# jturner65/distRayTracer_old

Measured on AMD Instinct MI355X. Metric: Mray/s + achieved HBM GB/s, bun69k.cli 1024² 16spp, 1/2/4/8 GPU, higher is better.
Workload: dtype f64

## Files before the change

distraytracer_old_amd/csrc/scene_build.cpp:

```cpp
#include <algorithm>
#include <cmath>
#include <map>
#include <string>

#include "host_math.h"
#include "rt_internal.h"

namespace rt {
using namespace hm;

namespace {

struct Box {
  double mn[3] = {100000, 100000, 100000};
  double mx[3] = {-100000, -100000, -100000};
};
static void calc_min_max(Box& b, const double* mn, const double* mx) {
  for (int i = 0; i < 3; ++i) { b.mn[i] = jmin(mn[i], b.mn[i]); b.mx[i] = jmax(mx[i], b.mx[i]); }
}
static void expand_pt(Box& b, D3 p) {
  double v[3] = {p.x, p.y, p.z};
  for (int i = 0; i < 3; ++i) {
    b.mn[i] = (b.mn[i] < v[i]) ? b.mn[i] : v[i];
    b.mx[i] = (b.mx[i] > v[i]) ? b.mx[i] : v[i];
// ... 451 lines not shown
        if (s.num_colors < 4) { err = "stone: needs at least 4 noise colours (mortar pair + a brick pair)"; return false; }
        md.distFunc = s.dist_func; md.roiFunc = s.roi_func; md.numPtsDist = s.num_pts_dist; md.mortar = s.mortar_thresh;
        std::map<double, int> pdfs;
        double lastDist = 1.0 / std::pow(M_E, s.avg_per_cell), cumProb = lastDist;
        for (int i = 1; i < 15; ++i) {
          lastDist *= (s.avg_per_cell / (1.0 * i));
          cumProb += lastDist;
          pdfs[cumProb] = i;
        }
        md.npdf = 0;
        for (auto& e : pdfs) { md.pdfKey[md.npdf] = e.first; md.pdfVal[md.npdf] = e.second; md.npdf++; }
      }
      hs.mat.push_back(md);
    }
    for (int l = 0; l < d->num_lights; ++l) {
      const rt_light_desc& s = d->lights[l];
      LightD ld;
      std::memset(&ld, 0, sizeof(ld));
      ld.type = s.type;
      ld.index = l;
      for (int c = 0; c < 3; ++c) { ld.origin[c] = s.pos[c]; ld.color[c] = s.color[c]; }
      D3 o = normalized(d3(s.dir[0], s.dir[1], s.dir[2]));
      ld.orient[0] = o.x; ld.orient[1] = o.y; ld.orient[2] = o.z;
      if (s.type != RT_LIGHT_POINT) {
        D3 t = ortho(o);
        ld.tangent[0] = t.x; ld.tangent[1] = t.y; ld.tangent[2] = t.z;
      }
      ld.innerRad = s.inner_deg * DEG_TO_RAD_F;
      ld.outerRad = s.outer_deg * DEG_TO_RAD_F;
      ld.radDiff = ld.outerRad - ld.innerRad;
      ld.radius = s.radius;
      std::memcpy(ld.g, s.ctm, sizeof(ld.g));
      {
        bool ident = true;
        for (int q = 0; q < 16; ++q) ident = ident && ld.g[q] == ((q % 5 == 0) ? 1.0 : 0.0);
        ld.pad[0] = (ident && (s.type == RT_LIGHT_POINT || s.type == RT_LIGHT_SPOT)) ? 1 : 0;
      }
      hs.light.push_back(ld);
    }
    int64_t off = 0;
    for (int t = 0; t < d->num_textures; ++t) {
      const rt_texture_desc& s = d->textures[t];
      if (s.w <= 0 || s.h <= 0 || !s.rgb) { err = "bad texture"; return false; }
      TexD td;
      td.w = s.w; td.h = s.h; td.off = off;
      hs.tex.push_back(td);
      for (int64_t k = 0; k < (int64_t)s.w * s.h; ++k)
        hs.texel.push_back(0xFF000000u | ((uint32_t)s.rgb[3 * k] << 16) | ((uint32_t)s.rgb[3 * k + 1] << 8) | s.rgb[3 * k + 2]);
      off += (int64_t)s.w * s.h;
    }
    if (d->bkg_texture >= d->num_textures) { err = "bad background texture"; return false; }
    hs.fov = d->fov;
    for (int c = 0; c < 3; ++c) hs.bg[c] = d->background[c];
    hs.bkgTex = d->bkg_texture;
    for (int c = 0; c < 4; ++c) hs.sky[c] = d->skydome[c];
    hs.dof = d->dof; hs.lensRadius = d->lens_radius; hs.lensFocal = d->lens_focal;
    if (d->camera < RT_CAMERA_FOV || d->camera > RT_CAMERA_ORTHO) { err = "bad camera type"; return false; }
    hs.camera = d->camera;
    hs.cameraParam[0] = d->camera_param[0]; hs.cameraParam[1] = d->camera_param[1];
    if (hs.camera != RT_CAMERA_FOV) hs.dof = 0;
    hs.rpp = d->rays_per_pixel;
    hs.photonMode = d->photon_mode; hs.photonCount = d->photon_count; hs.photonK = d->photon_k;
    hs.photonMaxD2 = d->photon_max_dist * d->photon_max_dist;
    return true;
  }
};

// ... 119 lines not shown
```

distraytracer_old_amd/csrc/trace_device.h:

```cpp
#pragma once
#include <hip/hip_runtime.h>
#include <stdint.h>

#include "rt_types.h"
#define QD_FN __device__ __forceinline__
#include "qdiv.h"

namespace rt {
namespace dv {

#define DEVI __device__ __forceinline__

static constexpr double EPS = 0.0000001;
static constexpr double DMAX = 1.7976931348623157e308;
static constexpr double TWO_PI_F = 6.2831854820251465;
static constexpr double PI_F = 3.1415927410125732;
static constexpr double PI_D = 3.141592653589793;

enum : uint32_t {
  SITE_AA_Y = 1, SITE_AA_X = 2, SITE_DOF_ANG = 3, SITE_DOF_RAD = 4, SITE_TIME = 8,
  SITE_DISK = 0x100, SITE_SHADOW_TIME = 0x200, SITE_PH_DIR = 0x1000, SITE_PH_BOUNCE = 0x1100, SITE_PH_TIME = 0x1200
};
enum { C_CAMERA = 0, C_SHADOW, C_REFL, C_REFR, C_BOX, C_TRI, C_QUAD, C_IMPLICIT, C_LIGHT, C_PHOTON, C_TEXEL,
       C_NODE, C_LEAF, C_MEMBER, C_ROOT, C_TOP,
       C_WNODE, C_WTRI, C_WQUAD, C_WIMPLICIT, C_WLIGHT, C_WPHOTON, C_N = 24 };

struct V {
  double x, y, z;
};
DEVI V mk(double x, double y, double z) { V r; r.x = x; r.y = y; r.z = z; return r; }
DEVI V sub(V a, V b) { return mk(a.x - b.x, a.y - b.y, a.z - b.z); }
DEVI V add(V a, V b) { return mk(a.x + b.x, a.y + b.y, a.z + b.z); }
DEVI V scl(V a, double s) { return mk(a.x * s, a.y * s, a.z * s); }
DEVI double dot(V a, V b) { return ((a.x * b.x) + (a.y * b.y)) + (a.z * b.z); }
DEVI V cross(V a, V b) { return mk((a.y * b.z) - (a.z * b.y), (a.z * b.x) - (a.x * b.z), (a.x * b.y) - (a.y * b.x)); }
DEVI double mag(V a) { return sqrt(((a.x * a.x) + (a.y * a.y)) + (a.z * a.z)); }
DEVI V nrmz(V a) {
  double m = mag(a);
  if (m == 0) return a;
  return mk(a.x / m, a.y / m, a.z / m);
}
DEVI bool veq(V a, V b) { return a.x == b.x && a.y == b.y && a.z == b.z; }
DEVI V ld3(const double* p) { return mk(p[0], p[1], p[2]); }
DEVI double jmin(double a, double b) { return (a != a) ? a : ((a <= b) ? a : b); }
DEVI double jmax(double a, double b) { return (a != a) ? a : ((a >= b) ? a : b); }
DEVI int32_t jd2i(double v) {
  if (v != v) return 0;
  if (v >= 2147483647.0) return 2147483647;
  if (v <= -2147483648.0) return (int32_t)0x80000000;
  return (int32_t)v;
}
DEVI V xpt(const double* m, V p) {
  double r[3];
#pragma unroll
  for (int row = 0; row < 3; ++row) {
    double a = 0.0;
    a += m[row * 4 + 0] * p.x;
    a += m[row * 4 + 1] * p.y;
    a += m[row * 4 + 2] * p.z;
    a += m[row * 4 + 3] * 1.0;
    r[row] = a;
  }
  return mk(r[0], r[1], r[2]);
}
DEVI V xvec(const double* m, V p) {
  double r[3];
#pragma unroll
  for (int row = 0; row < 3; ++row) {
    double a = 0.0;
    a += m[row * 4 + 0] * p.x;
    a += m[row * 4 + 1] * p.y;
    a += m[row * 4 + 2] * p.z;
    a += m[row * 4 + 3] * 0.0;
    r[row] = a;
  }
  return mk(r[0], r[1], r[2]);
}

DEVI uint64_t mix64(uint64_t z) {
  z += 0x9E3779B97F4A7C15ULL;
  z = (z ^ (z >> 30)) * 0xBF58476D1CE4E5B9ULL;
  z = (z ^ (z >> 27)) * 0x94D049BB133111EBULL;
  return z ^ (z >> 31);
}
DEVI double rng(uint64_t seed, uint64_t a, uint32_t b, uint32_t c, uint32_t site, uint32_t k, double lo, double hi) {
  uint64_t h = mix64(seed ^ mix64(a));
  h = mix64(h ^ (((uint64_t)b << 32) | c));
  h = mix64(h ^ (((uint64_t)site << 32) | k));
  double r = (double)(h >> 11) * 0x1.0p-53;
  r = r * (hi - lo) + lo;
  if (r >= hi) r = __longlong_as_double(__double_as_longlong(hi) - 1);
  return r;
}

struct Key {
  uint64_t seed, pixel;
  uint32_t sample, node;
  uint32_t tsite;
};

struct WRay {
  V o, d, d0;
  uint32_t ver;
  bool stable;
  bool moved;
};
DEVI void renorm(WRay& r) {
  if (!r.stable) {
    V n = nrmz(r.d);
    r.stable = veq(n, r.d);
    if (!r.stable) { r.moved = true; r.ver++; }
    r.d = n;
  }
}

#ifdef RT_PROF_PKSTAT
enum { P_CB_STEP = C_N, P_CB_LANES, P_CT_STEP, P_CT_LANES, P_AB_STEP, P_AB_LANES, P_AT_STEP, P_AT_LANES,
       P_RAY_STEP, P_RAY_LANES, P_SH_STEP, P_SH_LANES,
       P_CTH_STEP, P_CTH_LANES, P_ATH_STEP, P_ATH_LANES,
       P_N };
#else
enum { P_N = C_N };
#endif
struct Counters {
  uint64_t c[P_N];
};

struct RayInv {
  double y[3];
  bool fast;
};
DEVI RayInv ray_inv(V o, V d, int sceneOk) {
  RayInv r;
  r.y[0] = 1.0 / d.x; r.y[1] = 1.0 / d.y; r.y[2] = 1.0 / d.z;
  r.fast = sceneOk && qd_range(d.x) && qd_range(d.y) && qd_range(d.z) && qc_range(o.x) && qc_range(o.y) && qc_range(o.z);
  return r;
}

template <bool FAST>
DEVI bool slab_t(const double* mn, const double* mx, V o, V d, const double* y, double& tEntry) {
  double ro[3] = {o.x, o.y, o.z}, rd[3] = {d.x, d.y, d.z};
// ... 137 lines not shown
    if (r == 1) {
      const double g = (dist - te) - EPS, tol = APX * (fabs(te) + fabs(dist));
      if (g > tol) return true;
      if (-g > tol) return false;
    }
  }
  return slab_exact(mn, mx, o, d, ri, te) && (dist - te) > EPS;
}

DEVI int slab_plane(const double* mn, const double* mx, V o, V d) {
  double ro[3] = {o.x, o.y, o.z}, rd[3] = {d.x, d.y, d.z};
  double biggestMin = -DMAX;
  int idx = -1;
  for (int i = 0; i < 3; ++i) {
    double t1 = (mn[i] - ro[i]) / rd[i], t2 = (mx[i] - ro[i]) / rd[i];
    if (t1 < t2) { if (biggestMin < t1) { idx = i; biggestMin = t1; } }
    else { if (biggestMin < t2) { idx = i + 3; biggestMin = t2; } }
  }
  return idx;
}

struct LimNone {
  DEVI bool ok(double) const { return true; }
};
struct LimClosest {
  double a, b;
  DEVI bool ok(double t) const { return t < a || t < b; }
};
struct LimShadow {
  double dist;
  DEVI bool ok(double t) const { return (dist - t) > EPS; }
};

template <int NV, bool PLANE, class LIM = LimNone>
DEVI bool planar_test(const double (*v)[3], V nA, V nB, double dA, double dB, V o, V d, double& t, int& st,
                      const LIM& lim = LIM()) {
  double pr = dot(nA, d);
  if (!(fabs(pr) > 0)) return false;
  V N;
  double D;
  if (pr > 0) {
    pr = dot(nB, d);
    if (!(fabs(pr) > 0) || pr > 0) return false;
    N = nB; D = dB; st = 1;
  } else {
    N = nA; D = dA; st = 0;
  }
  t = -(dot(N, o) + D) / pr;
  if (!(t > EPS)) return false;
  if (PLANE) return true;
  if (!lim.ok(t)) return false;
  V p = mk(d.x * t + o.x, d.y * t + o.y, d.z * t + o.z);
#pragma unroll
  for (int i = 0; i < NV; ++i) {
    int vi = st ? (NV - 1 - i) : i;
    int pi = st ? (NV - 1 - (i == 0 ? NV - 1 : i - 1)) : (i == 0 ? NV - 1 : i - 1);
    V w = ld3(v[vi]), wp = ld3(v[pi]);
    V e = sub(w, wp);
    V ir = mk(p.x - w.x, p.y - w.y, p.z - w.z);
    if (dot(cross(ir, e), N) < -EPS) return false;
  }
  return true;
}

template <class LIM = LimNone, class TR = TriD>
DEVI bool tri_test(const TR& T, V o, V d, double& t, int& st, const LIM& lim = LIM()) {
  V nA = ld3(T.n);
  V nB = mk(-nA.x, -nA.y, -nA.z);
  return planar_test<3, false>(T.v, nA, nB, T.dA, T.dB, o, d, t, st, lim);
}

template <bool SL, class T>
DEVI T pld(const T* p) {
  if constexpr (SL) return *(const __attribute__((address_space(4))) T*)p;
  else return *p;
}
template <bool SL>
DEVI V pld3(const double* p) { return mk(pld<SL>(p), pld<SL>(p + 1), pld<SL>(p + 2)); }

template <bool SL = false>
DEVI V sphere_center(const PrimD& P, const Key& k) {
  if (pld<SL>(&P.type) != PT_MSPHERE) return pld3<SL>(P.a);
  double tm = rng(k.seed, k.pixel, k.sample, k.node, k.tsite, pld<SL>(&P.key), 0, 1.0);
  V o0 = pld3<SL>(P.a), o1 = pld3<SL>(P.a + 6);
  V bMa = sub(o1, o0);
  return mk(o0.x + tm * bMa.x, o0.y + tm * bMa.y, o0.z + tm * bMa.z);
}

template <bool SL = false>
DEVI bool prim_test(const PrimD& P, V o, V d, const Key& k, double& t, int& args) {
  const int32_t type = pld<SL>(&P.type);
  auto A = [&](int i) { return pld<SL>(P.a + i); };
  switch (type) {
    case PT_QUAD:
    case PT_PLANE: {
      if constexpr (SL) {
        double q[4][3];
#pragma unroll
        for (int i = 0; i < 12; ++i) q[i / 3][i % 3] = A(i);
        if (type == PT_PLANE)
          return planar_test<4, true>(q, pld3<SL>(P.a + 12), pld3<SL>(P.a + 15), A(18), A(19), o, d, t, args);
        return planar_test<4, false>(q, pld3<SL>(P.a + 12), pld3<SL>(P.a + 15), A(18), A(19), o, d, t, args);
// ... 110 lines not shown
```

distraytracer_old_amd/csrc/trace_kernels.h:

```cpp
#pragma once
#include "trace_device.h"
#include "jfdlibm.h"

namespace rt {
namespace dv {

enum : uint32_t {
  FT_PRIM = 1,
  FT_TEX = 2,
  FT_PHOTON = 4,
  FT_TRANS = 8,
  FT_DOF = 16,
  FT_LIGHTX = 32,
  FT_CAMX = 64,
  FT_INST = 128,
  FT_PASS = 256,
  FT_CELL = 512,
  FT_ALL = 1023
};

static __constant__ int c_perm[256];
static __constant__ int c_grad3[12][3];

struct Best {
  double t;
  int32_t ref;
  uint32_t ver;
  int16_t top;
  int16_t inAcc;
  int32_t inst;
  uint32_t iver;
};
DEVI Best miss() { Best b; b.t = DMAX; b.ref = 0; b.top = -1; b.ver = 0; b.inAcc = 0; b.inst = -1; b.iver = 0; return b; }
struct HitCtx {
  int32_t top, inst;
  uint32_t wver;
};

#define WCNT(idx, n)                                                                      \
  do {                                                                                    \
    if (CNT && __lane_id() == (int)__builtin_ctzll(__ballot(1))) ct.c[idx] += (n);        \
  } while (0)
#ifndef RT_ULOAD
#define RT_ULOAD 1
#endif
#ifndef RT_SPRIM
#define RT_SPRIM 2
#endif
template <uint32_t F>
static constexpr bool SPRIM = RT_SPRIM == 2 || (RT_SPRIM == 1 && (F & FT_PHOTON) == 0);
template <bool CNT, uint32_t F, class LIM = LimNone, bool WAVE = false>
DEVI bool test_ref(const SceneD& S, int32_t ref, V o, V d, const Key& k, double& t, int& args, Counters& ct,
                   const LIM& lim = LIM()) {
  if (!(F & FT_PRIM) || ref >= 0) {
    if (CNT) ct.c[C_TRI]++;
    if (WAVE) WCNT(C_WTRI, 1); else if (CNT) ct.c[C_WTRI]++;
    return tri_test(S.tri[ref], o, d, t, args, lim);
  }
  const PrimD& P = S.prim[~ref];
  if (CNT) {
    const int c = (P.type == PT_QUAD || P.type == PT_PLANE) ? C_QUAD : C_IMPLICIT;
    ct.c[c]++;
    if (WAVE) WCNT(c + (C_WQUAD - C_QUAD), 1); else ct.c[c + (C_WQUAD - C_QUAD)]++;
  }
  return prim_test<WAVE && SPRIM<F>>(P, o, d, k, t, args);
}
template <uint32_t F>
DEVI int32_t ref_xf(const SceneD& S, int32_t ref) { return (!(F & FT_PRIM) || ref >= 0) ? S.tri[ref].xf : S.prim[~ref].xf; }

template <class T>
DEVI T sload(const T* p) {
  static_assert(sizeof(T) == 4 || sizeof(T) == 8, "scalar field");
  return *(const __attribute__((address_space(4))) T*)p;
}
struct ChildBox {
  double mn[3], mx[3];
  int32_t ref;
};
DEVI ChildBox sload_child(const NodeD* nd, int side) {
  ChildBox c;
  const double* b = side ? nd->rmin : nd->lmin;
#pragma unroll
  for (int i = 0; i < 3; ++i) { c.mn[i] = sload(b + i); c.mx[i] = sload(b + 3 + i); }
  c.ref = sload(side ? &nd->right : &nd->left);
  return c;
}
struct TriG {
  double v[3][3];
  double n[3];
  double dA, dB;
// ... 120 lines not shown
#pragma unroll
  for (int i = 0; i < 9; ++i) t.m[i] = sload(&p->m[0][0] + i);
#pragma unroll
  for (int i = 0; i < 3; ++i) { t.c[i] = sload(p->c + i); t.n[i] = sload(p->n + i); }
  t.d = sload(&p->d); t.k = sload(&p->k); t.tm = sload(&p->tm);
  return t;
}
static constexpr float EPS_F32_UP = 1.00000001168609742e-07f;
DEVI bool tri_f32_out(const TriFR& T, const TriRayF& r) {
  const float s = __builtin_fmaf(T.n[2], r.d[2], __builtin_fmaf(T.n[1], r.d[1], T.n[0] * r.d[0]));
  const float P = __builtin_fmaf(T.n[2], r.o[2], __builtin_fmaf(T.n[1], r.o[1], __builtin_fmaf(T.n[0], r.o[0], T.d)));
  const float as = fabsf(s), sP = s < 0 ? -P : P;
  const float B = __builtin_fmaf(r.D, __builtin_fmaf(T.k, r.O + T.tm, 0x1p-40f), 0x1p-100f);
  const float thr = -__builtin_fmaf(EPS_F32_UP, as, B);
  bool out = false;
#pragma unroll
  for (int j = 0; j < 3; ++j) {
    const float* m = T.m + 3 * j;
    const float Q = __builtin_fmaf(m[2], r.o[2], __builtin_fmaf(m[1], r.o[1], __builtin_fmaf(m[0], r.o[0], -T.c[j])));
    const float R = __builtin_fmaf(m[2], r.d[2], __builtin_fmaf(m[1], r.d[1], m[0] * r.d[0]));
    out = out || (__builtin_fmaf(as, Q, -(sP * R)) < thr);
  }
  return out && as > 0x1p-20f * r.D && B < 0x1p100f;
}

template <bool CNT, uint32_t F, bool PK, class LIM = LimNone>
DEVI bool test_ref_u(const SceneD& S, int32_t ref, V o, V d, const Key& k, double& t, int& args, Counters& ct,
                     const LIM& lim = LIM()) {
  if constexpr (PK) {
    if (!(F & FT_PRIM) || ref >= 0) {
      if (CNT) ct.c[C_TRI]++;
      WCNT(C_WTRI, 1);
      const TriG T = sload_tri(S.tri + ref);
      return tri_test(T, o, d, t, args, lim);
    }
  }
  return test_ref<CNT, F, LIM, PK>(S, ref, o, d, k, t, args, ct, lim);
}
template <uint32_t F, bool PK>
DEVI int32_t ref_xf_u(const SceneD& S, int32_t ref) {
  if (PK && (!(F & FT_PRIM) || ref >= 0)) return sload(&S.tri[ref].xf);
  return ref_xf<F>(S, ref);
}
template <uint32_t F>
DEVI bool is_inst(const SceneD& S, int32_t ref) { return (F & FT_INST) && ref < 0 && S.prim[~ref].type == PT_INST; }


struct LeafR {
  int32_t start, count;
  bool run;
};
template <bool PK = false>
DEVI LeafR leaf_of(const SceneD& S, int32_t c) {
  LeafR r;
  r.run = (c & LEAF_RUN_FLAG) != 0;
  if (r.run) { r.start = (c >> 5) & LEAF_RUN_MAXSTART; r.count = c & 31; }
  else if (PK) { r.start = sload(&S.leaf[c].start); r.count = sload(&S.leaf[c].count); }
  else { LeafD lf = S.leaf[c]; r.start = lf.start; r.count = lf.count; }
  return r;
}
template <bool PK = false>
DEVI int32_t leaf_member(const SceneD& S, const LeafR& lf, int i) {
  return lf.run ? lf.start + i : (PK ? sload(S.member + lf.start + i) : S.member[lf.start + i]);
}

template <bool CNT, uint32_t F>
DEVI void inst_closest(const SceneD& S, int32_t ii, WRay& w, const Key& k, int top, Best& best, double& local, Counters& ct);

template <bool CNT, uint32_t F, bool INST, bool PK = false>
DEVI void leaf_closest(const SceneD& S, int32_t leaf, int accXf, V ao, V ad, WRay& w, const Key& k, const HitCtx& hc,
                       Best& best, double& local, Counters& ct) {
  const LeafR lf = leaf_of<PK>(S, leaf);
  if (CNT) { ct.c[C_LEAF]++; ct.c[C_MEMBER] += lf.count; }
  constexpr bool TF32 = PK && !INST && RT_F32_TRI != 0 && RT_F32_TRI_CPK != 0 &&
                        ((F & FT_PHOTON) == 0 || RT_F32_TRI_PH_CPK != 0);
  TriRayF trf;
  if constexpr (TF32) trf = tri_ray_f32(ao, ad);
  for (int i = 0; i < lf.count; ++i) {
    if (PK) PKSTAT(P_CT_STEP, __ballot(1));
    int32_t ref = leaf_member<PK>(S, lf, i);
    renorm(w);
    if constexpr (!INST && (F & FT_INST) != 0) {
      if (is_inst<F>(S, ref)) {
        inst_closest<CNT, F>(S, ~ref, w, k, hc.top, best, local, ct);
        continue;
      }
    }
    int xf = ref_xf_u<F, PK>(S, ref);
    V o, d;
    if (xf == accXf && !w.moved) { o = ao; d = ad; }
    else if (PK && (RT_ULOAD & 1)) {
      double inv[12];
      sload_inv(S.xf + xf, inv);
      o = xpt(inv, w.o); d = xvec(inv, w.d);
    } else { const double* inv = S.xf[xf].inv; o = xpt(inv, w.o); d = xvec(inv, w.d); }
    double t;
    int args;
    bool th;
    if (TF32 && (!(F & FT_PRIM) || ref >= 0) && xf == accXf && !w.moved) {
      if (CNT) ct.c[C_TRI]++;
      WCNT(C_WTRI, 1);
      const TriFR TF = sload_trif(S.triF + ref);
      th = false;
      if (!tri_f32_out(TF, trf)) {
        const TriG T = sload_tri(S.tri + ref);
        th = tri_test(T, o, d, t, args, LimClosest{local, best.t});
      }
    } else {
      th = test_ref_u<CNT, F, PK>(S, ref, o, d, k, t, args, ct, LimClosest{local, best.t});
    }
    if (th) {
      if (t < local) local = t;
      if (t < best.t) {
        best.t = t; best.ref = ref; best.top = (int16_t)hc.top; best.inAcc = 1; best.inst = hc.inst;
        if (INST) { best.ver = hc.wver; best.iver = w.ver; }
        else { best.ver = w.ver; best.iver = 0; }
      }
    }
  }
}

static constexpr int BVH_STACK = 40;

#ifndef RT_STACK_LDS
#define RT_STACK_LDS 12
#endif
static constexpr int STK_LDS = RT_STACK_LDS;
extern __shared__ double rt_lds[];
static constexpr int LDS_STACK_BYTES = STK_LDS * 64 * 12;
#ifndef RT_PK_LDS
#define RT_PK_LDS 16
#endif
static constexpr int PK_LDS = RT_PK_LDS;
static constexpr int PKO_M = PK_LDS * 64 * 8;
static constexpr int PKO_R = PKO_M + BVH_STACK * 8;
static constexpr int PKO_N = PKO_R + BVH_STACK * 8;
static constexpr int PKO_C = PKO_N + BVH_STACK * 4;
static constexpr int LDS_PK_BYTES = PKO_C + BVH_STACK * 4;
static constexpr int LDS_MAX2 = LDS_STACK_BYTES > LDS_PK_BYTES ? LDS_STACK_BYTES : LDS_PK_BYTES;
// ... 488 lines not shown
        act = nearLeft ? L : R;
      } else if (L) {
        cur = cl; act = L;
      } else if (R) {
        cur = cr; act = R;
      } else {
        N = INT32_MAX;
      }
      if (N != INT32_MAX) { N = cur.ref; continue; }
#endif
    } else {
      const int32_t c = ~N;
      const int32_t st = (c >> 5) & LEAF_RUN_MAXSTART, cnt = c & 31;
      if (CNT && in_mask_t<MASKOPS<F>>(act)) { ct.c[C_LEAF]++; ct.c[C_MEMBER] += cnt; }
#if RT_F32_TRI
      const TriRayF trf = tri_ray_f32(ao, ad);
#endif
      for (int i = 0; i < cnt; ++i) {
        PKSTAT(P_CT_STEP, act);
        WCNT(C_WTRI, 1);
        bool need = in_mask_t<MASKOPS<F>>(act);
        if (CNT && need) ct.c[C_TRI]++;
#if RT_F32_TRI
        {
          const TriFR TF = sload_trif(S.triF + st + i);
          if (need) need = !tri_f32_out(TF, trf);
          if (!__ballot(need)) continue;
        }
#endif
        const TriG T = sload_tri(S.tri + st + i);
        if (need) {
          double t;
          int args;
          const bool th = tri_test(T, ao, ad, t, args, LimNF{bt, best.t});
          PKSTAT_HIT(P_CTH_STEP, th);
          if (th && (t < bt || (t == bt && st + i < bref))) {
            bt = t;
            bref = st + i;
            double te;
#if RT_NF_CODE
            const ChildBox cur = sload_child(S.node + (curCode >> 1), curCode & 1);
#endif
            inside = slab_exact(cur.mn, cur.mx, ao, ad, ri, te) && te < t - t * 0x1p-40;
          }
        }
      }
    }
    N = INT32_MAX;
    while (sp > 0) {
      --sp;
      const int32_t code = uni(pkN()[sp]);
      uint64_t M = uni64(pkM()[sp]);
      const NodeD* pn = S.node + (code >> 1);
      bool keep = false;
      if (in_mask_t<MASKOPS<F>>(M)) {
        const double bnd = fmin(best.t, bt), lim = fmin(bnd + bnd * 0x1p-40, 0x1p1000);
        double e;
        if (sp < PK_LDS) {
          e = pkT()[sp * 64 + __lane_id()];
        } else {
          const ChildBox cb = sload_child(pn, code & 1);
          e = entry_grown(cb.mn, cb.mx, sload_slack(pn, code & 1), ao, ri.y);
        }
        keep = e <= lim;
      }
      M = __ballot(keep);
#if RT_NF_CODE
// ... 130 lines not shown
DEVI void step_cands_all() {
  for (int q = 0; q < GRP_MAX; ++q) wcM()[q] = ~0ull;
}
DEVI uint64_t step_cand(int li) { return li < GRP_MAX ? uni64(*(volatile lds_u64*)(wcM() + li)) : ~0ull; }

#ifndef RT_PACKET
#define RT_PACKET 1
#endif
static constexpr bool PACKET = RT_PACKET != 0;
#ifndef RT_STASH_SHADE
#define RT_STASH_SHADE 1
#endif
static constexpr bool STASH_SHADE = PACKET && RT_STASH_SHADE != 0 && PK_LDS >= SL_N;
#ifndef RT_LANE_DIV
#define RT_LANE_DIV 0
#endif
#ifndef RT_LANE_DIV_COS
#define RT_LANE_DIV_COS 0.9
#endif
template <bool CNT, uint32_t F, bool PK = false>
DEVI Best closest(const SceneD& S, WRay& w, const Key& k, Counters& ct) {
  PROF_T0(t_all);
  Best best = miss();
  bool lanes = false;
  if constexpr (PK && RT_LANE_DIV > 0) {
    const int f = (int)__builtin_ctzll(__ballot(1));
    const double c = w.d.x * rdl(w.d.x, f) + w.d.y * rdl(w.d.y, f) + w.d.z * rdl(w.d.z, f);
    const int nfar = __popcll(__ballot(!(c >= RT_LANE_DIV_COS))), nact = __popcll(__ballot(1));
    lanes = RT_LANE_DIV == 1 ? (nfar >= 2 && 2 * nfar >= nact) : nfar >= RT_LANE_DIV;
  }
  for (int i = 0; i < S.ntop; ++i) {
    TopD tp = PK ? sload_top(S.top + i) : S.top[i];
    if (CNT) ct.c[C_TOP]++;
    renorm(w);
    if ((F & FT_INST) && tp.kind == TOP_INST) {
      double local = best.t;
      inst_closest<CNT, F>(S, tp.idx, w, k, i, best, local, ct);
      continue;
    }
    if ((((F & FT_PRIM) && tp.kind == TOP_PRIM) || (tp.kind == TOP_ACCEL && w.stable)) && top_culled<PK>(S, i, w, best.t))
      continue;
    V o, d;
    if (PK) {
      double inv[12];
      sload_inv(S.xf + tp.xf, inv);
      o = xpt(inv, w.o); d = xvec(inv, w.d);
    } else {
      const double* inv = S.xf[tp.xf].inv;
      o = xpt(inv, w.o); d = xvec(inv, w.d);
    }
    if (tp.kind == TOP_ACCEL) {
      const AccelD A = PK ? sload_accel(S.accel + tp.idx) : S.accel[tp.idx];
      if (CNT) { ct.c[C_ROOT]++; ct.c[C_BOX]++; }
      RayInv ri = ray_inv(o, d, S.fastSlab & SCENE_FAST_SLAB);
      if (!box_hit<MASKOPS<F>>(A.bmin, A.bmax, o, d, ri)) continue;
      w.moved = false;
      double local = DMAX;
      PROF_T0(t_acc);
      if (RT_LANE_DIV > 0 && lanes)
        accel_closest<CNT, F, false>(S, A, o, d, ri, w, k, HitCtx{i, -1, 0}, best, local, ct);
      else if (PK && NEAREST_FIRST && (F & (FT_PHOTON | (RT_NF_TRANS ? 0 : FT_TRANS))) == 0 && (S.fastSlab & SCENE_NEAREST_FIRST) &&
          (A.flags & ACCEL_NEAREST) &&
          !__ballot(!(w.stable && ri.fast)))
        accel_closest_nf<CNT, F>(S, A, o, d, ri, w, k, HitCtx{i, -1, 0}, best, local, ct);
      else if (PK) accel_closest_pk<CNT, F>(S, A, o, d, ri, w, k, HitCtx{i, -1, 0}, best, local, ct);
      else accel_closest<CNT, F, false>(S, A, o, d, ri, w, k, HitCtx{i, -1, 0}, best, local, ct);
      PROF_ADD(t_acc, R_CLOSEST_ACCEL);
    } else {
      int32_t ref = tp.kind == TOP_TRI ? tp.idx : ~tp.idx;
      double t;
      int args;
      if (test_ref_u<CNT, F, PK>(S, ref, o, d, k, t, args, ct, LimClosest{best.t, best.t}) && t < best.t) {
        best.t = t; best.ref = ref; best.top = (int16_t)i; best.inAcc = 0; best.ver = w.ver; best.inst = -1; best.iver = 0;
      }
    }
  }
  PROF_ADD(t_all, R_CLOSEST);
  return best;
}

template <bool CNT, bool A2 = (RT_APX2 != 0)>
DEVI bool shadow_box(const double* mn, const double* mx, V o, V d, const RayInv& ri, double dist, Counters& ct) {
  if (CNT) ct.c[C_BOX]++;
  return box_shadow<A2>(mn, mx, o, d, ri, dist);
}
template <bool CNT, uint32_t F>
DEVI bool inst_any(const SceneD& S, int32_t ii, const WRay& w, const Key& k, double dist, Counters& ct);

template <bool CNT, uint32_t F, bool INST, bool PK = false>
DEVI bool leaf_any(const SceneD& S, int32_t leaf, int accXf, V ao, V ad, WRay& w, const Key& k, double dist, Counters& ct) {
  const LeafR lf = leaf_of<PK>(S, leaf);
  if (CNT) { ct.c[C_LEAF]++; ct.c[C_MEMBER] += lf.count; }
  constexpr bool TF32 = PK && RT_F32_TRI != 0 && ((F & FT_PHOTON) == 0 || RT_F32_TRI_PH_ANY != 0);
  TriRayF trf;
  if constexpr (TF32) trf = tri_ray_f32(ao, ad);
  for (int i = 0; i < lf.count; ++i) {
    if (PK) PKSTAT(P_AT_STEP, __ballot(1));
    int32_t ref = leaf_member<PK>(S, lf, i);
    renorm(w);
    if constexpr (!INST && (F & FT_INST) != 0) {
      if (is_inst<F>(S, ref)) {
        if (inst_any<CNT, F>(S, ~ref, w, k, dist, ct)) return true;
        continue;
      }
    }
    int xf = ref_xf_u<F, PK>(S, ref);
    V o, d;
    if (xf == accXf && !w.moved) { o = ao; d = ad; }
    else if (PK && (RT_ULOAD & 1)) {
      double inv[12];
      sload_inv(S.xf + xf, inv);
      o = xpt(inv, w.o); d = xvec(inv, w.d);
    } else { const double* inv = S.xf[xf].inv; o = xpt(inv, w.o); d = xvec(inv, w.d); }
    double t;
    int args;
    bool th;
    if (TF32 && (!(F & FT_PRIM) || ref >= 0) && xf == accXf && !w.moved) {
      if (CNT) ct.c[C_TRI]++;
      WCNT(C_WTRI, 1);
      const TriFR TF = sload_trif(S.triF + ref);
      th = false;
      if (!tri_f32_out(TF, trf)) {
        const TriG T = sload_tri(S.tri + ref);
        th = tri_test(T, o, d, t, args, LimShadow{dist}) && (dist - t) > EPS;
      }
    } else {
      th = test_ref_u<CNT, F, PK>(S, ref, o, d, k, t, args, ct, LimShadow{dist}) && (dist - t) > EPS;
    }
    if (PK) PKSTAT_HIT(P_ATH_STEP, th);
    if (th) return true;
  }
  return false;
}
template <bool CNT, uint32_t F, bool INST>
DEVI bool accel_any(const SceneD& S, const AccelD& A, V ao, V ad, WRay& w, const Key& k, double dist, Counters& ct) {
  RayInv ri = ray_inv(ao, ad, S.fastSlab & SCENE_FAST_SLAB);
  NStackT<INST ? 0 : STK_LDS> st;
  int sp = 0;
  int32_t N = A.root;
  if (N < 0 && !shadow_box<CNT>(A.bmin, A.bmax, ao, ad, ri, dist, ct)) return false;
  while (true) {
    if (N >= 0) {
      const NodeD& nd = S.node[N];
      if (CNT) { ct.c[C_NODE]++; ct.c[C_WNODE]++; }
      st.setN(sp++, N);
      if (shadow_box<CNT>(nd.lmin, nd.lmax, ao, ad, ri, dist, ct)) { N = nd.left; continue; }
    } else if (N != INT32_MAX) {
      if (leaf_any<CNT, F, INST>(S, ~N, INST ? -1 : A.xf, ao, ad, w, k, dist, ct)) return true;
      if (INST && w.moved) { ad = w.d; ri = ray_inv(ao, ad, S.fastSlab & SCENE_FAST_SLAB); w.moved = false; }
    }
    N = INT32_MAX;
    while (sp > 0) {
      const NodeD& pn = S.node[st.getN(--sp)];
      if (shadow_box<CNT>(pn.rmin, pn.rmax, ao, ad, ri, dist, ct)) { N = pn.right; break; }
    }
    if (N == INT32_MAX) return false;
  }
// ... 104 lines not shown
      --sp;
      if (CNT && in_mask_t<MASKOPS<F>>(st.getM(sp) & alive)) ct.c[C_BOX]++;
      const uint64_t R = st.getR(sp) & alive;
      if (R) { act = R; N = st.getC(sp); break; }
    }
    if (N == INT32_MAX) return blocked;
  }
}

template <bool CNT, uint32_t F>
DEVI bool inst_any(const SceneD& S, int32_t ii, const WRay& w, const Key& k, double dist, Counters& ct) {
  if constexpr ((F & FT_INST) != 0) {
    const PrimD& I = S.prim[ii];
    const double* inv = S.xf[I.xf].inv;
    WRay wi;
    wi.o = xpt(inv, w.o);
    wi.d = xvec(inv, w.d);
    wi.d0 = wi.d;
    wi.ver = 0; wi.stable = false; wi.moved = false;
    if (I.flags & PF_INST_ACCEL) return accel_any<CNT, F, true>(S, S.accel[I.pad[0]], wi.o, wi.d, wi, k, dist, ct);
    double t;
    int args;
    return test_ref<CNT, F>(S, I.pad[0], wi.o, wi.d, k, t, args, ct, LimShadow{dist}) && (dist - t) > EPS;
  }
  return false;
}
template <bool CNT, uint32_t F, bool PK = false, bool WC = false>
DEVI bool shadowed_(const SceneD& S, WRay& w, const Key& k, double dist, Counters& ct, int li) {
  const uint64_t cand = WC ? step_cand(li) : ~0ull;
  for (int i = 0; i < S.ntop; ++i) {
    if (WC && i < 64) {
      const uint64_t rest = cand & (~0ull << i);
      const int nx = rest ? (int)__builtin_ctzll(rest) : S.ntop;
      for (int j = i; j < nx && !w.stable; ++j) renorm(w);
      if (nx >= S.ntop) break;
      i = nx;
    }
    TopD tp = PK ? sload_top(S.top + i) : S.top[i];
    if (CNT) ct.c[C_TOP]++;
#if defined(RT_PROF_SH_NOQUAD) || defined(RT_PROF_SH_NOIMPL)
    if (tp.kind == TOP_PRIM) {
      const bool bounded = sload(S.topBound + 4 * i + 3) > 0;
#ifdef RT_PROF_SH_NOQUAD
      if (!bounded) continue;
#else
      if (bounded) continue;
#endif
    }
#endif
#ifdef RT_PROF_SH_NOACCEL
    if (tp.kind == TOP_ACCEL) continue;
#endif
    renorm(w);
    if ((F & FT_INST) && tp.kind == TOP_INST) {
      if (inst_any<CNT, F>(S, tp.idx, w, k, dist, ct)) return true;
      continue;
    }
    if ((((F & FT_PRIM) && tp.kind == TOP_PRIM) || (tp.kind == TOP_ACCEL && w.stable)) && top_culled<PK>(S, i, w, dist))
      continue;
#ifdef RT_PROF_SH_SCANONLY
    continue;
#endif
    V o, d;
    if (PK) {
      double inv[12];
      sload_inv(S.xf + tp.xf, inv);
      o = xpt(inv, w.o); d = xvec(inv, w.d);
    } else {
      const double* inv = S.xf[tp.xf].inv;
      o = xpt(inv, w.o); d = xvec(inv, w.d);
    }
    if (tp.kind == TOP_ACCEL) {
      if (CNT) ct.c[C_ROOT]++;
      w.moved = false;
      PROF_T0(t_acc);
      const bool blk = PK ? accel_any_pk<CNT, F>(S, sload_accel(S.accel + tp.idx), o, d, w, k, dist, ct)
                          : accel_any<CNT, F, false>(S, S.accel[tp.idx], o, d, w, k, dist, ct);
      PROF_ADD(t_acc, R_SHADOW_ACCEL);
      if (blk) return true;
    } else {
      int32_t ref = tp.kind == TOP_TRI ? tp.idx : ~tp.idx;
      double t;
      int args;
      if (test_ref_u<CNT, F, PK>(S, ref, o, d, k, t, args, ct, LimShadow{dist}) && (dist - t) > EPS) return true;
    }
  }
  return false;
}
#ifdef RT_SHADOW_NOINLINE
#define SHADOW_FN __device__ __attribute__((noinline))
#else
#define SHADOW_FN DEVI
#endif
template <bool CNT, uint32_t F, bool PK = false, bool WC = false>
SHADOW_FN bool shadowed(const SceneD& S, WRay& w, const Key& k, double dist, Counters& ct, int li = 0) {
  PROF_T0(t_all);
  const bool r = shadowed_<CNT, F, PK, WC>(S, w, k, dist, ct, li);
  PROF_ADD(t_all, R_SHADOW);
  return r;
}

struct HitRec {
  V hitLoc, fwd, nrm, dw;
  int32_t mat, args, type, ref;
  uint32_t key;
};
template <uint32_t F>
DEVI HitRec make_hit(const SceneD& S, const Best& b, const WRay& w, const Key& k) {
  HitRec h;
  int32_t ref = b.ref;
  V dw = w.d0;
  for (uint32_t i = 0; i < b.ver; ++i) dw = nrmz(dw);
  int xf, xfc;
  if (!(F & FT_PRIM) || ref >= 0) { const TriD& T = S.tri[ref]; xf = T.xf; xfc = T.xfc; h.mat = T.mat; h.key = T.key; h.type = PT_TRI; }
  else { const PrimD& P = S.prim[~ref]; xf = P.xf; xfc = P.xfc; h.mat = P.mat; h.key = P.key; h.type = P.type; }
  h.ref = ref;
  V ro = w.o;
  int hitXf = -1;
  bool direct = false;
  if ((F & FT_INST) && b.inst >= 0) {
    const PrimD& I = S.prim[b.inst];
    const XformD& XI = S.xf[I.xf];
    ro = xpt(XI.inv, w.o);
    dw = xvec(XI.inv, dw);
    for (uint32_t i = 0; i < b.iver; ++i) dw = nrmz(dw);
    if (I.mat >= 0) h.mat = I.mat;
    direct = !(I.flags & PF_INST_ACCEL);
    hitXf = (I.xfc >= 0) ? I.xfc : (direct ? I.xf : -1);
  }
  const XformD& X = S.xf[xf];
  V tro = direct ? ro : xpt(X.inv, ro), trd = direct ? dw : xvec(X.inv, dw);
  double t = b.t, tt;
  int args = 0;
  if (!(F & FT_PRIM) || ref >= 0) {
    const V nA = ld3(S.tri[ref].n);
    args = dot(nA, trd) > 0 ? 1 : 0;
  } else {
    Counters dummy;
    test_ref<false, F>(S, ref, tro, trd, k, tt, args, dummy);
  }
  h.args = args;
  V p = mk(trd.x * t + tro.x, trd.y * t + tro.y, trd.z * t + tro.z);
  h.hitLoc = p;
  V n;
  if (!(F & FT_PRIM) || ref >= 0) {
// ... 978 lines not shown

__device__ __attribute__((noinline)) double pow_call(double x, double e) { return pow(x, e); }
DEVI double pow_shade(double x, double e) {
  if (!(e >= 0 && e <= 1024 && e == floor(e))) return pow_call(x, e);
  int n = (int)e;
  double r = 1, b = x;
  while (n) {
    if (n & 1) r *= b;
    n >>= 1;
    if (n) b *= b;
  }
  return r;
}
template <bool CNT, uint32_t F, bool STASH>
DEVI V light_sum(const SceneD& S, const MatD& m, const HitRec& h, V tex, const Key& k, Counters& ct) {
  double r = 0, g = 0, b = 0;
  if (STASH) stash3(SL_RGB, mk(0, 0, 0));
  if constexpr (WAVE_CULL<F>) {
    if (S.fastSlab & SCENE_WAVE_CULL) step_cands(S, h.fwd);
    else step_cands_all();
  }
  for (int li = 0; li < S.nlight; ++li) {
    if (STASH) lds_barrier();
    const LightD& L = S.light[li];
    const int32_t ltype = sload(&L.type);
    double lg[12];
#pragma unroll
    for (int q = 0; q < 12; ++q) lg[q] = sload(L.g + q);
    const V lorg = mk(sload(L.origin), sload(L.origin + 1), sload(L.origin + 2));
    const V lcol = mk(sload(L.color), sload(L.color + 1), sload(L.color + 2));
    const bool disk = (F & FT_LIGHTX) && ltype == 2;
    V lo = disk ? disk_pos<(RT_ULOAD & 2) != 0>(L, k, 0) : lorg;
    V ln = xpt(lg, lo);
    ln = nrmz(mk(ln.x - h.fwd.x, ln.y - h.fwd.y, ln.z - h.fwd.z));
    WRay sr;
    sr.o = h.fwd;
    sr.d = nrmz(ln);
    sr.d0 = sr.d;
    sr.stable = false;
    sr.moved = false;
    sr.ver = 0;
    V lo2 = disk ? disk_pos<(RT_ULOAD & 2) != 0>(L, k, 2) : lorg;
    double t = sqrt((((sr.o.x - lo2.x) * (sr.o.x - lo2.x)) + ((sr.o.y - lo2.y) * (sr.o.y - lo2.y))) + ((sr.o.z - lo2.z) * (sr.o.z - lo2.z)));
    double ltMult = 1;
    if (CNT) ct.c[C_LIGHT]++;
    WCNT(C_WLIGHT, 1);
    if ((F & FT_LIGHTX) && ltype == 1) {
      constexpr bool U = (RT_ULOAD & 2) != 0;
      double angle = jf::acos(-1 * dot(sr.d, pld3<U>(L.orient)));
      const double inR = pld<U>(&L.innerRad), outR = pld<U>(&L.outerRad);
      ltMult = (angle < inR) ? 1 : (angle > outR) ? 0 : (outR - angle) / pld<U>(&L.radDiff);
    }
    if (ltMult == 0) continue;
    if (CNT) ct.c[C_SHADOW]++;
    Key sk = k;
    sk.tsite = SITE_SHADOW_TIME + li;
    PKSTAT(P_SH_STEP, __ballot(1));
    if (STASH && (F & FT_LIGHTX)) { stash(SL_LTM, ltMult); lds_barrier(); }
#ifdef RT_PROF_NOSHADOW
    if (false)
#endif
    if (shadowed<CNT, F, PACKET, WAVE_CULL<F>>(S, sr, sk, t, ct, li)) continue;
    renorm(sr);
    if (STASH) {
      if (F & FT_LIGHTX) ltMult = unstash(SL_LTM);
      const V rgb = unstash3(SL_RGB);
      r = rgb.x; g = rgb.y; b = rgb.z;
    }
    const V hn = STASH ? unstash3(SL_NRM) : h.nrm;
    double ldp = dot(sr.d, hn) * ltMult;
    if (ldp > EPS) {
      const V tx = STASH ? unstash3(SL_TEX) : tex;
      r += tx.x * lcol.x * ldp;
      g += tx.y * lcol.y * ldp;
      b += tx.z * lcol.z * ldp;
    }
    if (STASH) stash3(SL_RGB, mk(r, g, b));
#ifdef RT_PROF_NOPHONG
    continue;
#endif
    if (m.phong == 0) continue;
    const V hdw = STASH ? unstash3(SL_DW) : h.dw;
    const V hv = mk(sr.d.x - hdw.x, sr.d.y - hdw.y, sr.d.z - hdw.z);
    const double hm = mag(hv), hr = hm == 0 ? 1.0 : 1.0 / hm;
    double hdp = (hv.x * hr * hn.x + hv.y * hr * hn.y + hv.z * hr * hn.z) * ltMult;
    if (hdp > EPS) {
      double ph = pow_shade(hdp * hdp, m.phong);
      r += m.specular[0] * lcol.x * ph;
      g += m.specular[1] * lcol.y * ph;
      b += m.specular[2] * lcol.z * ph;
      if (STASH) stash3(SL_RGB, mk(r, g, b));
    }
  }
  if (STASH) { lds_barrier(); return unstash3(SL_RGB); }
  return mk(r, g, b);
}
// ... 351 lines not shown
  for (int w = 32; w >= 1; w >>= 1) {
    const int c = __popcll(m & ((1ull << w) - 1));
    if (r >= c) { r -= c; m >>= w; pos += w; }
  }
  return pos;
}
DEVI double key_pack(const Key& k) {
  return __builtin_bit_cast(double, (uint64_t)(uint32_t)k.pixel | ((uint64_t)(k.sample & 0xFFFFFu) << 32) |
                                        ((uint64_t)(k.node & 0xFFFu) << 52));
}
DEVI Key key_unpack(double v, uint64_t seed, uint32_t tsite) {
  const uint64_t b = __builtin_bit_cast(uint64_t, v);
  Key k;
  k.seed = seed; k.pixel = (uint32_t)b; k.sample = (uint32_t)(b >> 32) & 0xFFFFFu; k.node = (uint32_t)(b >> 52);
  k.tsite = tsite;
  return k;
}
struct ShRay {
  V d;
  double dist, ltm;
};
template <uint32_t F, bool U>
DEVI ShRay shadow_ray(const SceneD& S, int li, V fwd, const Key& k) {
  const LightD& L = S.light[li];
  auto ld = [&](const double* p) { return U ? sload(p) : *p; };
  const int32_t ltype = U ? sload(&L.type) : L.type;
  double lg[12];
#pragma unroll
  for (int q = 0; q < 12; ++q) lg[q] = ld(L.g + q);
  const V lorg = mk(ld(L.origin), ld(L.origin + 1), ld(L.origin + 2));
  const bool disk = (F & FT_LIGHTX) && ltype == 2;
  const V lo = disk ? disk_pos<U>(L, k, 0) : lorg;
  V ln = xpt(lg, lo);
  ln = nrmz(mk(ln.x - fwd.x, ln.y - fwd.y, ln.z - fwd.z));
  ShRay r;
  r.d = nrmz(ln);
  const V lo2 = disk ? disk_pos<U>(L, k, 2) : lorg;
  r.dist = sqrt((((fwd.x - lo2.x) * (fwd.x - lo2.x)) + ((fwd.y - lo2.y) * (fwd.y - lo2.y))) +
                ((fwd.z - lo2.z) * (fwd.z - lo2.z)));
  r.ltm = 1;
  if ((F & FT_LIGHTX) && ltype == 1) {
    const double angle = jf::acos(-1 * dot(r.d, pld3<U>(L.orient)));
    const double inR = pld<U>(&L.innerRad), outR = pld<U>(&L.outerRad);
    r.ltm = (angle < inR) ? 1 : (angle > outR) ? 0 : (outR - angle) / pld<U>(&L.radDiff);
  }
  return r;
}
template <bool CNT, uint32_t F>
DEVI V light_sum_w(const SceneD& S, bool hit, int32_t mat, const Key& k, Counters& ct) {
  if (!__ballot(hit)) return mk(0, 0, 0);
  const int lane = __lane_id();
  double r = 0, g = 0, b = 0;
  lds_u64* gm = grpM();
  int li0 = 0, ns = 0, n = 0;
  const int nl = S.nlight;
  for (int li = 0; li <= nl; ++li) {
    uint64_t mask = 0;
    if (li < nl) {
      double ltm = 0;
      if (hit) {
        if (CNT) ct.c[C_LIGHT]++;
        ltm = shadow_ray<F, true>(S, li, unstash3(SL_FWD), k).ltm;
        if (CNT && ltm != 0) ct.c[C_SHADOW]++;
      }
      WCNT(C_WLIGHT, 1);
      mask = __ballot(hit && ltm != 0);
    }
    const int c = __popcll(mask);
    if (li == nl || n + c > 64 || ns == GRP_MAX) {
      if (n > 0) {
        lds_barrier();
        int es = 0, er = 0, base = 0;
        for (int s = 0; s < ns; ++s) {
          const int cs = __popcll(uni64(gm[s]));
          if (lane >= base && lane < base + cs) { es = s; er = lane - base; }
          base += cs;
        }
        int res = -1;
        if (lane < n) {
          const int src = nth_bit(gm[es], er);
          const V o = mk(pkT()[SL_FWD * 64 + src], pkT()[(SL_FWD + 1) * 64 + src], pkT()[(SL_FWD + 2) * 64 + src]);
          const Key sk = key_unpack(pkT()[SL_KEY * 64 + src], k.seed, SITE_SHADOW_TIME + li0 + es);
          const ShRay sh = shadow_ray<F, false>(S, li0 + es, o, sk);
          WRay sr;
          sr.o = o; sr.d = sh.d; sr.d0 = sh.d; sr.stable = false; sr.moved = false; sr.ver = 0;
          PKSTAT(P_SH_STEP, __ballot(1));
          PROF_T0(t_shd);
#ifdef RT_PROF_NOSHADOW
          if (true) {
#else
          if (!shadowed<CNT, F, PACKET>(S, sr, sk, sh.dist, ct)) {
#endif
            renorm(sr);
            res = (int)sr.ver;
          }
          PROF_ADD(t_shd, R_SHADOW);
        }
        lds_barrier();
        const uint64_t below = lanes_below();
        base = 0;
        for (int s = 0; s < ns; ++s) {
          const uint64_t m = uni64(gm[s]);
          const int rs = __builtin_amdgcn_ds_bpermute((base + (int)__popcll(m & below)) << 2, res);
          base += __popcll(m);
          if (in_mask(m) && rs >= 0) {
            const int lj = li0 + s;
            const ShRay sh = shadow_ray<F, true>(S, lj, unstash3(SL_FWD), k);
            V d = sh.d;
            for (int q = 0; q < rs; ++q) d = nrmz(d);
            const LightD& L = S.light[lj];
            const V lcol = mk(sload(L.color), sload(L.color + 1), sload(L.color + 2));
            const V hn = unstash3(SL_NRM);
            const double ldp = dot(d, hn) * sh.ltm;
            if (ldp > EPS) {
              const V tx = unstash3(SL_TEX);
              r += tx.x * lcol.x * ldp;
              g += tx.y * lcol.y * ldp;
              b += tx.z * lcol.z * ldp;
            }
#ifndef RT_PROF_NOPHONG
            const MatD& mt = S.mat[mat];
            if (mt.phong != 0) {
              const V hdw = unstash3(SL_DW);
              const V hv = mk(d.x - hdw.x, d.y - hdw.y, d.z - hdw.z);
              const double hm = mag(hv), hr = hm == 0 ? 1.0 : 1.0 / hm;
              const double hdp = (hv.x * hr * hn.x + hv.y * hr * hn.y + hv.z * hr * hn.z) * sh.ltm;
// ... 776 lines not shown
```

Before: 16170.

## Skip redundant normalization, distance and plane work for scenes without transforms or prims

Adds compile-time specializations, active when the scene has no transforms or primitives, that remove redundant double-precision work. Renormalization is skipped when the squared length is exactly one. Triangle tests reject early when the plane numerator has the wrong sign. make_hit reuses the already-normalized direction when the versions match, and for identity-transformed point and spot lights the shadow distance reuses the magnitude computed during normalization. Each shortcut must reproduce the original bit-exact results, so any mismatch in version counting or rounding could change the image.

```diff
diff --git a/distraytracer_old_amd/csrc/scene_build.cpp b/distraytracer_old_amd/csrc/scene_build.cpp
--- a/distraytracer_old_amd/csrc/scene_build.cpp
+++ b/distraytracer_old_amd/csrc/scene_build.cpp
@@ -507,7 +507,7 @@
       ld.radius = s.radius;
       std::memcpy(ld.g, s.ctm, sizeof(ld.g));
       {
-        bool ident = true;
+        bool ident = std::isfinite(ld.origin[0]) && std::isfinite(ld.origin[1]) && std::isfinite(ld.origin[2]);
         for (int q = 0; q < 16; ++q) ident = ident && ld.g[q] == ((q % 5 == 0) ? 1.0 : 0.0);
         ld.pad[0] = (ident && (s.type == RT_LIGHT_POINT || s.type == RT_LIGHT_SPOT)) ? 1 : 0;
       }
diff --git a/distraytracer_old_amd/csrc/trace_device.h b/distraytracer_old_amd/csrc/trace_device.h
--- a/distraytracer_old_amd/csrc/trace_device.h
+++ b/distraytracer_old_amd/csrc/trace_device.h
@@ -40,6 +40,15 @@
   if (m == 0) return a;
   return mk(a.x / m, a.y / m, a.z / m);
 }
+DEVI V nrmz_m(V a, double& m) {
+  m = mag(a);
+  if (m == 0) return a;
+  return mk(a.x / m, a.y / m, a.z / m);
+}
+DEVI bool unit_len(V a) {
+  const double s = ((a.x * a.x) + (a.y * a.y)) + (a.z * a.z);
+  return s == 1.0 || s == 1.0 + 0x1p-52;
+}
 DEVI bool veq(V a, V b) { return a.x == b.x && a.y == b.y && a.z == b.z; }
 DEVI V ld3(const double* p) { return mk(p[0], p[1], p[2]); }
 DEVI double jmin(double a, double b) { return (a != a) ? a : ((a <= b) ? a : b); }
@@ -105,8 +114,13 @@
   bool stable;
   bool moved;
 };
+#ifndef RT_RENORM_UNIT
+#define RT_RENORM_UNIT 1
+#endif
+template <bool UNIT>
 DEVI void renorm(WRay& r) {
   if (!r.stable) {
+    if (UNIT && unit_len(r.d)) { r.stable = true; return; }
     V n = nrmz(r.d);
     r.stable = veq(n, r.d);
     if (!r.stable) { r.moved = true; r.ver++; }
@@ -310,7 +324,10 @@
   DEVI bool ok(double t) const { return (dist - t) > EPS; }
 };
 
-template <int NV, bool PLANE, class LIM = LimNone>
+#ifndef RT_PLANAR_SIGN
+#define RT_PLANAR_SIGN 1
+#endif
+template <int NV, bool PLANE, bool SIGN = false, class LIM = LimNone>
 DEVI bool planar_test(const double (*v)[3], V nA, V nB, double dA, double dB, V o, V d, double& t, int& st,
                       const LIM& lim = LIM()) {
   double pr = dot(nA, d);
@@ -324,7 +341,9 @@
   } else {
     N = nA; D = dA; st = 0;
   }
-  t = -(dot(N, o) + D) / pr;
+  const double num = dot(N, o) + D;
+  if (SIGN && !(num > 0)) return false;
+  t = -num / pr;
   if (!(t > EPS)) return false;
   if (PLANE) return true;
   if (!lim.ok(t)) return false;
@@ -341,11 +360,11 @@
   return true;
 }
 
-template <class LIM = LimNone, class TR = TriD>
+template <bool SIGN, class LIM = LimNone, class TR = TriD>
 DEVI bool tri_test(const TR& T, V o, V d, double& t, int& st, const LIM& lim = LIM()) {
   V nA = ld3(T.n);
   V nB = mk(-nA.x, -nA.y, -nA.z);
-  return planar_test<3, false>(T.v, nA, nB, T.dA, T.dB, o, d, t, st, lim);
+  return planar_test<3, false, SIGN>(T.v, nA, nB, T.dA, T.dB, o, d, t, st, lim);
 }
 
 template <bool SL, class T>
diff --git a/distraytracer_old_amd/csrc/trace_kernels.h b/distraytracer_old_amd/csrc/trace_kernels.h
--- a/distraytracer_old_amd/csrc/trace_kernels.h
+++ b/distraytracer_old_amd/csrc/trace_kernels.h
@@ -18,6 +18,19 @@
   FT_CELL = 512,
   FT_ALL = 1023
 };
+
+#ifndef RT_HIT_DW
+#define RT_HIT_DW 1
+#endif
+#ifndef RT_LIGHT_DIST
+#define RT_LIGHT_DIST 1
+#endif
+template <uint32_t F>
+constexpr bool known_norm() { return (F & (FT_TRANS | FT_PRIM)) == 0; }
+template <uint32_t F> static constexpr bool KN_UNIT = RT_RENORM_UNIT != 0 && known_norm<F>();
+template <uint32_t F> static constexpr bool KN_SIGN = RT_PLANAR_SIGN != 0 && known_norm<F>();
+template <uint32_t F> static constexpr bool KN_DW = RT_HIT_DW != 0 && known_norm<F>();
+template <uint32_t F> static constexpr bool KN_DIST = RT_LIGHT_DIST != 0 && known_norm<F>();
 
 static __constant__ int c_perm[256];
 static __constant__ int c_grad3[12][3];
@@ -55,7 +68,7 @@
   if (!(F & FT_PRIM) || ref >= 0) {
     if (CNT) ct.c[C_TRI]++;
     if (WAVE) WCNT(C_WTRI, 1); else if (CNT) ct.c[C_WTRI]++;
-    return tri_test(S.tri[ref], o, d, t, args, lim);
+    return tri_test<KN_SIGN<F>>(S.tri[ref], o, d, t, args, lim);
   }
   const PrimD& P = S.prim[~ref];
   if (CNT) {
@@ -242,7 +255,7 @@
       if (CNT) ct.c[C_TRI]++;
       WCNT(C_WTRI, 1);
       const TriG T = sload_tri(S.tri + ref);
-      return tri_test(T, o, d, t, args, lim);
+      return tri_test<KN_SIGN<F>>(T, o, d, t, args, lim);
     }
   }
   return test_ref<CNT, F, LIM, PK>(S, ref, o, d, k, t, args, ct, lim);
@@ -289,7 +302,7 @@
   for (int i = 0; i < lf.count; ++i) {
     if (PK) PKSTAT(P_CT_STEP, __ballot(1));
     int32_t ref = leaf_member<PK>(S, lf, i);
-    renorm(w);
+    renorm<KN_UNIT<F>>(w);
     if constexpr (!INST && (F & FT_INST) != 0) {
       if (is_inst<F>(S, ref)) {
         inst_closest<CNT, F>(S, ~ref, w, k, hc.top, best, local, ct);
@@ -314,7 +327,7 @@
       th = false;
       if (!tri_f32_out(TF, trf)) {
         const TriG T = sload_tri(S.tri + ref);
-        th = tri_test(T, o, d, t, args, LimClosest{local, best.t});
+        th = tri_test<KN_SIGN<F>>(T, o, d, t, args, LimClosest{local, best.t});
       }
     } else {
       th = test_ref_u<CNT, F, PK>(S, ref, o, d, k, t, args, ct, LimClosest{local, best.t});
@@ -869,7 +882,7 @@
         if (need) {
           double t;
           int args;
-          const bool th = tri_test(T, ao, ad, t, args, LimNF{bt, best.t});
+          const bool th = tri_test<KN_SIGN<F>>(T, ao, ad, t, args, LimNF{bt, best.t});
           PKSTAT_HIT(P_CTH_STEP, th);
           if (th && (t < bt || (t == bt && st + i < bref))) {
             bt = t;
@@ -1066,7 +1079,7 @@
   for (int i = 0; i < S.ntop; ++i) {
     TopD tp = PK ? sload_top(S.top + i) : S.top[i];
     if (CNT) ct.c[C_TOP]++;
-    renorm(w);
+    renorm<KN_UNIT<F>>(w);
     if ((F & FT_INST) && tp.kind == TOP_INST) {
       double local = best.t;
       inst_closest<CNT, F>(S, tp.idx, w, k, i, best, local, ct);
@@ -1131,7 +1144,7 @@
   for (int i = 0; i < lf.count; ++i) {
     if (PK) PKSTAT(P_AT_STEP, __ballot(1));
     int32_t ref = leaf_member<PK>(S, lf, i);
-    renorm(w);
+    renorm<KN_UNIT<F>>(w);
     if constexpr (!INST && (F & FT_INST) != 0) {
       if (is_inst<F>(S, ref)) {
         if (inst_any<CNT, F>(S, ~ref, w, k, dist, ct)) return true;
@@ -1156,7 +1169,7 @@
       th = false;
       if (!tri_f32_out(TF, trf)) {
         const TriG T = sload_tri(S.tri + ref);
-        th = tri_test(T, o, d, t, args, LimShadow{dist}) && (dist - t) > EPS;
+        th = tri_test<KN_SIGN<F>>(T, o, d, t, args, LimShadow{dist}) && (dist - t) > EPS;
       }
     } else {
       th = test_ref_u<CNT, F, PK>(S, ref, o, d, k, t, args, ct, LimShadow{dist}) && (dist - t) > EPS;
@@ -1327,7 +1340,7 @@
     if (WC && i < 64) {
       const uint64_t rest = cand & (~0ull << i);
       const int nx = rest ? (int)__builtin_ctzll(rest) : S.ntop;
-      for (int j = i; j < nx && !w.stable; ++j) renorm(w);
+      for (int j = i; j < nx && !w.stable; ++j) renorm<KN_UNIT<F>>(w);
       if (nx >= S.ntop) break;
       i = nx;
     }
@@ -1346,7 +1359,7 @@
 #ifdef RT_PROF_SH_NOACCEL
     if (tp.kind == TOP_ACCEL) continue;
 #endif
-    renorm(w);
+    renorm<KN_UNIT<F>>(w);
     if ((F & FT_INST) && tp.kind == TOP_INST) {
       if (inst_any<CNT, F>(S, tp.idx, w, k, dist, ct)) return true;
       continue;
@@ -1404,8 +1417,11 @@
 DEVI HitRec make_hit(const SceneD& S, const Best& b, const WRay& w, const Key& k) {
   HitRec h;
   int32_t ref = b.ref;
-  V dw = w.d0;
-  for (uint32_t i = 0; i < b.ver; ++i) dw = nrmz(dw);
+  V dw = w.d;
+  if (!KN_DW<F> || b.ver != w.ver) {
+    dw = w.d0;
+    for (uint32_t i = 0; i < b.ver; ++i) dw = nrmz(dw);
+  }
   int xf, xfc;
   if (!(F & FT_PRIM) || ref >= 0) { const TriD& T = S.tri[ref]; xf = T.xf; xfc = T.xfc; h.mat = T.mat; h.key = T.key; h.type = PT_TRI; }
   else { const PrimD& P = S.prim[~ref]; xf = P.xf; xfc = P.xfc; h.mat = P.mat; h.key = P.key; h.type = P.type; }
@@ -2450,7 +2466,8 @@
     const bool disk = (F & FT_LIGHTX) && ltype == 2;
     V lo = disk ? disk_pos<(RT_ULOAD & 2) != 0>(L, k, 0) : lorg;
     V ln = xpt(lg, lo);
-    ln = nrmz(mk(ln.x - h.fwd.x, ln.y - h.fwd.y, ln.z - h.fwd.z));
+    double lm;
+    ln = nrmz_m(mk(ln.x - h.fwd.x, ln.y - h.fwd.y, ln.z - h.fwd.z), lm);
     WRay sr;
     sr.o = h.fwd;
     sr.d = nrmz(ln);
@@ -2458,8 +2475,13 @@
     sr.stable = false;
     sr.moved = false;
     sr.ver = 0;
-    V lo2 = disk ? disk_pos<(RT_ULOAD & 2) != 0>(L, k, 2) : lorg;
-    double t = sqrt((((sr.o.x - lo2.x) * (sr.o.x - lo2.x)) + ((sr.o.y - lo2.y) * (sr.o.y - lo2.y))) + ((sr.o.z - lo2.z) * (sr.o.z - lo2.z)));
+    double t;
+    if (KN_DIST<F> && sload(&L.pad[0]) == 1) {
+      t = lm;
+    } else {
+      V lo2 = disk ? disk_pos<(RT_ULOAD & 2) != 0>(L, k, 2) : lorg;
+      t = sqrt((((sr.o.x - lo2.x) * (sr.o.x - lo2.x)) + ((sr.o.y - lo2.y) * (sr.o.y - lo2.y))) + ((sr.o.z - lo2.z) * (sr.o.z - lo2.z)));
+    }
     double ltMult = 1;
     if (CNT) ct.c[C_LIGHT]++;
     WCNT(C_WLIGHT, 1);
@@ -2479,7 +2501,7 @@
     if (false)
 #endif
     if (shadowed<CNT, F, PACKET, WAVE_CULL<F>>(S, sr, sk, t, ct, li)) continue;
-    renorm(sr);
+    renorm<KN_UNIT<F>>(sr);
     if (STASH) {
       if (F & FT_LIGHTX) ltMult = unstash(SL_LTM);
       const V rgb = unstash3(SL_RGB);
@@ -2897,12 +2919,17 @@
   const bool disk = (F & FT_LIGHTX) && ltype == 2;
   const V lo = disk ? disk_pos<U>(L, k, 0) : lorg;
   V ln = xpt(lg, lo);
-  ln = nrmz(mk(ln.x - fwd.x, ln.y - fwd.y, ln.z - fwd.z));
+  double lm;
+  ln = nrmz_m(mk(ln.x - fwd.x, ln.y - fwd.y, ln.z - fwd.z), lm);
   ShRay r;
   r.d = nrmz(ln);
-  const V lo2 = disk ? disk_pos<U>(L, k, 2) : lorg;
-  r.dist = sqrt((((fwd.x - lo2.x) * (fwd.x - lo2.x)) + ((fwd.y - lo2.y) * (fwd.y - lo2.y))) +
-                ((fwd.z - lo2.z) * (fwd.z - lo2.z)));
+  if (KN_DIST<F> && (U ? sload(&L.pad[0]) : L.pad[0]) == 1) {
+    r.dist = lm;
+  } else {
+    const V lo2 = disk ? disk_pos<U>(L, k, 2) : lorg;
+    r.dist = sqrt((((fwd.x - lo2.x) * (fwd.x - lo2.x)) + ((fwd.y - lo2.y) * (fwd.y - lo2.y))) +
+                  ((fwd.z - lo2.z) * (fwd.z - lo2.z)));
+  }
   r.ltm = 1;
   if ((F & FT_LIGHTX) && ltype == 1) {
     const double angle = jf::acos(-1 * dot(r.d, pld3<U>(L.orient)));
@@ -2956,7 +2983,7 @@
 #else
           if (!shadowed<CNT, F, PACKET>(S, sr, sk, sh.dist, ct)) {
 #endif
-            renorm(sr);
+            renorm<KN_UNIT<F>>(sr);
             res = (int)sr.ver;
           }
           PROF_ADD(t_shd, R_SHADOW);
```

Result: faster. 16690 (median of 6 runs) (+3.2%).
